# jesselasse/MARL-DMFB

Hardware: AMD Instinct MI355X
Metric: env-steps/sec (whole node), 10x10 DMFB 4-droplet fov9 (higher is better)
Workload: dtype int8 env state/obs + f64 rewards; fp32 Q-net; 1 GPU; DMFB 10x10, drop_num=4, fov=9, 4096 parallel envs per GPU (BASELINE configs[1]); parallelism=dp1: chips sharded per rank, one flat RCCL all-reduce per learn

## Files before the change

### marl_dmfb_amd/csrc/crnn_mfma.h

```cpp
#pragma once
#include <hip/hip_runtime.h>

#include <cstdint>

namespace crnn_mfma {

typedef float f32x4 __attribute__((ext_vector_type(4)));

constexpr int kBlockM = 512;

#ifdef CRNN_PROBE_TS
__device__ unsigned long long *g_crnn_ts;
#define CRNN_TS(k) do { if (lane == 0 && ts_it == 1 && g_crnn_ts) g_crnn_ts[((size_t)blockIdx.x * 8 + wave) * 16 + (k)] = __builtin_readcyclecounter(); } while (0)
#else
#define CRNN_TS(k) do { } while (0)
#endif

template <int OD, int RBV = 0, int NW = 8> struct GeoM {
    static constexpr int RB = RBV ? RBV : (OD <= 24 ? 16 : 12);
    static constexpr int CS = 53;
#ifdef CRNN_NO_ROWLANE
    static constexpr bool ROWLANE = false;
#else
    static constexpr bool ROWLANE = RB == 16;
#endif
    static constexpr int ROW_A1 = ROWLANE ? (OD * CS + 31) / 32 * 32 + 2 : OD * CS;
    static constexpr int IN_STRIDE = ROWLANE ? 258 : 244;
    static constexpr int PAD_COLS = (OD * 25 + 10 + 63) / 64 * 64;
    static constexpr int OUT_STRIDE = PAD_COLS + 4;
    static constexpr int KQ = OD / 4;
    static constexpr int NSTEP2 = KQ * 9;
    static constexpr int M1 = RB * 49, M2 = RB * 25;
    static constexpr int T2 = (M2 + 15) / 16;
    static constexpr int NSUB = NW / 2;
    static constexpr int BLOCK = 64 * NW;
    static_assert(NW == 8 || NW == 4, "wave roles");
    static_assert(RB % NSUB == 0 && RB <= 16, "conv1 tiling: rows split over NSUB waves per half, one position-48 tile");
    static constexpr int VEC = 18;
    static constexpr int MLP = 10 * VEC + 10;
    static constexpr size_t LDS_FLOATS = (size_t)RB * IN_STRIDE + (size_t)RB * ROW_A1 + (size_t)RB * OUT_STRIDE + (size_t)RB * VEC + MLP;
};

template <int OD, int RBV, int NT>
__device__ __forceinline__ void conv2_tiles(const float *s_a1, float *s_out, const float (&bw2)[GeoM<OD, RBV>::NSTEP2], float bias2,
                                            int t0, int t1, int j, int kq, int ch, bool chv) {
    using G = GeoM<OD, RBV>;
    const float *ap[NT];
    f32x4 acc[NT];
#pragma unroll
    for (int n = 0; n < NT; ++n) {
        int r, p;
        if constexpr (G::ROWLANE) {
            r = j;
            p = n == 0 ? t0 : t1;
        } else {
            int m = (n == 0 ? t0 : t1) * 16 + j;
            m = m < G::M2 ? m : G::M2 - 1;
            r = m / 25;
            p = m - r * 25;
        }
        ap[n] = s_a1 + r * G::ROW_A1 + (p / 5) * 7 + p % 5 + kq * G::CS;
        acc[n] = f32x4{bias2, bias2, bias2, bias2};
    }
    float v[2][NT][9];
#pragma unroll
    for (int tap = 0; tap < 9; ++tap)
#pragma unroll
        for (int n = 0; n < NT; ++n) v[0][n][tap] = ap[n][(tap / 3) * 7 + tap % 3];
#ifdef CRNN_PROBE_NO_GATHER
#define CRNN_GATHER(x) (bias2)
#else
#define CRNN_GATHER(x) (x)
#endif
#pragma unroll
    for (int cq = 0; cq < G::KQ; ++cq) {
        if (cq + 1 < G::KQ) {
#pragma unroll
            for (int tap = 0; tap < 9; ++tap)
#pragma unroll
                for (int n = 0; n < NT; ++n)
                    v[(cq + 1) & 1][n][tap] = CRNN_GATHER(ap[n][(cq + 1) * 4 * G::CS + (tap / 3) * 7 + tap % 3]);
        }
        __builtin_amdgcn_sched_barrier(0);
#pragma unroll
        for (int tap = 0; tap < 9; ++tap)
#pragma unroll
            for (int n = 0; n < NT; ++n)
                acc[n] = __builtin_amdgcn_mfma_f32_16x16x4f32(v[cq & 1][n][tap], bw2[cq * 9 + tap], acc[n], 0, 0, 0);
        __builtin_amdgcn_sched_barrier(0);
    }
#ifdef CRNN_PROBE_NO_EPI
    if (chv && acc[0][0] == 12345.678f) {
#else
    if (chv) {
#endif
#pragma unroll
        for (int n = 0; n < NT; ++n)
#pragma unroll
            for (int q = 0; q < 4; ++q) {
                if constexpr (G::ROWLANE) {
                    s_out[(kq * 4 + q) * G::OUT_STRIDE + ch * 25 + (n == 0 ? t0 : t1)] = fmaxf(acc[n][q], 0.0f);
                } else {
                    const int mm = (n == 0 ? t0 : t1) * 16 + kq * 4 + q;
                    if (mm < G::M2) { const int rr = mm / 25, pp = mm - rr * 25; s_out[rr * G::OUT_STRIDE + ch * 25 + pp] = fmaxf(acc[n][q], 0.0f); }
                }
            }
    }
}

template <int OD, int RBV = 0, int NW = 8>
__global__ __launch_bounds__(64 * NW) void k_conv9_mfma(const int8_t *__restrict__ obs, long obs_stride, long rows,
                                                        const float *__restrict__ w1, const float *__restrict__ b1,
                                                        const float *__restrict__ w2, const float *__restrict__ b2,
                                                        float *__restrict__ out, long out_stride, int out_cols,
                                                        const int8_t *__restrict__ onehot, int n_actions,
                                                        const float *__restrict__ mlp_w, const float *__restrict__ mlp_b,
                                                        const int32_t *__restrict__ live_chips, const int32_t *__restrict__ n_live,
                                                        int rows_per_chip) {
    using G = GeoM<OD, RBV, NW>;
    constexpr int kBlockM = G::BLOCK;
    extern __shared__ __attribute__((aligned(16))) float lds[];
    float *s_in = lds;
    float *s_a1 = s_in + G::RB * G::IN_STRIDE;
    float *s_out = s_a1 + G::RB * G::ROW_A1;
    float *s_vec = s_out + G::RB * G::OUT_STRIDE;
    float *s_mlp = s_vec + G::RB * G::VEC;
    const int tid = threadIdx.x, lane = tid & 63, wave = tid >> 6;
    const int nh = (wave >> 1) & 1, sub = (wave & 1) + 2 * (wave >> 2);
    const int j = lane & 15, kq = lane >> 4;
    const int ch = nh * 16 + j;
    const bool chv = ch < OD;

    if (live_chips) rows = min(rows, (long)n_live[0] * rows_per_chip);
    const long n_blocks = (rows + G::RB - 1) / G::RB;
    const int nin = 2 + n_actions;
    if (mlp_w) {
        for (int i = tid; i < 10 * nin; i += kBlockM) s_mlp[i] = mlp_w[i];
        if (tid < 10) s_mlp[10 * G::VEC + tid] = mlp_b[tid];
    }
    const uint32_t rpc = (uint32_t)(rows_per_chip > 0 ? rows_per_chip : 1);
    const uint32_t rpc_magic = rpc > 1 ? (uint32_t)(0x100000000ull / rpc) + 1u : 0u;
    auto src_row = [&](long cr) -> long {
        if (!live_chips) return cr;
        const uint32_t k = rpc > 1 ? __umulhi((uint32_t)cr, rpc_magic) : (uint32_t)cr;
        return (long)((uint32_t)live_chips[k] * rpc + ((uint32_t)cr - k * rpc));
    };
    constexpr int RPW = (G::RB + NW - 1) / NW, ROWB = 245;
    const int wave_u = __builtin_amdgcn_readfirstlane(wave);
    int pf[RPW][4], pfo[RPW];
    int pf_rv = 0;
#pragma unroll
    for (int h = 0; h < RPW; ++h) {
        pfo[h] = 0;
#pragma unroll
        for (int v = 0; v < 4; ++v) pf[h][v] = 0;
    }
    const int p3 = min(lane + 192, mlp_w ? ROWB - 1 : 242);
    auto fetch = [&](long b) {
        const long r0 = b * G::RB;
        pf_rv = b < n_blocks ? (int)min((long)G::RB, rows - r0) : 0;
#pragma unroll
        for (int h = 0; h < RPW; ++h) {
            const int rr = wave_u + NW * h;
            if (rr < pf_rv) {
                const long sr = src_row(r0 + rr);
                const int8_t *row = obs + sr * obs_stride;
                pf[h][0] = row[lane];
                pf[h][1] = row[lane + 64];
                pf[h][2] = row[lane + 128];
                pf[h][3] = row[p3];
                if (mlp_w && onehot && n_actions > 0) pfo[h] = onehot[sr * n_actions + min(lane, n_actions - 1)];
            }
        }
    };
    auto park = [&]() {
#pragma unroll
        for (int h = 0; h < RPW; ++h) {
            const int rr = wave_u + NW * h;
            if (rr < G::RB) {
                const bool on = rr < pf_rv;
                float *dst = s_in + rr * G::IN_STRIDE;
#pragma unroll
                for (int v = 0; v < 3; ++v) dst[lane + 64 * v] = on ? (float)pf[h][v] : 0.0f;
                const float last = on ? (float)pf[h][3] : 0.0f;
                if (lane + 192 < 243) dst[lane + 192] = last;
                else if (lane + 192 < ROWB) s_vec[rr * G::VEC + lane + 192 - 243] = last;
                if (lane < 16) s_vec[rr * G::VEC + 2 + lane] = (on && onehot && lane < n_actions) ? (float)pfo[h] : 0.0f;
            }
        }
    };
    fetch(blockIdx.x);

    for (int i = tid; i < OD * OD * 9; i += kBlockM) s_a1[i] = w2[i];
    for (int i = tid; i < OD * 27; i += kBlockM) s_in[i] = w1[i];
    __syncthreads();
    float bw1[7];
    int off1[7];
#pragma unroll
    for (int s = 0; s < 7; ++s) {
        const int k = 4 * s + kq;
        const bool kv = k < 27;
        bw1[s] = (chv && kv) ? s_in[ch * 27 + k] : 0.0f;
        const int c0 = k / 9, tap = k - c0 * 9;
        off1[s] = kv ? c0 * 81 + (tap / 3) * 9 + tap % 3 : (G::ROWLANE ? 1 : 0);
    }
    int goff[3];
#pragma unroll
    for (int qt = 0; qt < 3; ++qt) { const int p = qt * 16 + j; goff[qt] = (p / 7) * 9 + p % 7; }
    float bw2[G::NSTEP2];
#pragma unroll
    for (int cq = 0; cq < G::KQ; ++cq)
#pragma unroll
        for (int tap = 0; tap < 9; ++tap) bw2[cq * 9 + tap] = chv ? s_a1[(ch * OD + 4 * cq + kq) * 9 + tap] : 0.0f;
    __syncthreads();
    const float bias1 = chv ? b1[ch] : 0.0f, bias2 = chv ? b2[ch] : 0.0f;
    const int n_feat = OD * 25 + (mlp_w ? 10 : 0);
    const int n_out = out_cols > n_feat ? out_cols : n_feat;
    const bool wide_out = (out_stride % 2 == 0) && (((size_t)out) % 8 == 0) && (n_out % 2 == 0);
    const bool quad_out = (out_stride % 4 == 0) && (((size_t)out) % 16 == 0) && (n_out % 4 == 0) && (G::OUT_STRIDE % 4 == 0);
    for (int i = tid; i < G::RB * (G::OUT_STRIDE - n_feat); i += kBlockM) {
        const int rr = i / (G::OUT_STRIDE - n_feat), k = i - rr * (G::OUT_STRIDE - n_feat);
        s_out[rr * G::OUT_STRIDE + n_feat + k] = 0.0f;
    }

    park();
    __syncthreads();
#ifdef CRNN_PROBE_TS
    int ts_it = 0;
#endif
    for (long blk = blockIdx.x; blk < n_blocks; blk += gridDim.x) {
        CRNN_TS(0);
        const long row0 = blk * G::RB;
        const int rv = (int)min((long)G::RB, rows - row0);
        float mv = 0.0f;
        const int mr = tid / 10, mc = tid - mr * 10;
        if (mlp_w && tid < G::RB * 10) {
            mv = s_mlp[10 * G::VEC + mc];
            for (int k = 0; k < nin; ++k) mv = fmaf(s_vec[mr * G::VEC + k], s_mlp[mc * nin + k], mv);
        }
        fetch(blk + gridDim.x);
        CRNN_TS(1);
#ifndef CRNN_PROBE_SKIP_CONV1
        if constexpr (G::ROWLANE) {
            constexpr int NT1 = 49, NIT = (NT1 / G::NSUB) / 3;
            static_assert(G::NSUB == 4 && NIT * 3 * G::NSUB == NT1 - 1, "conv1 row-lane tiling");
            const int sub_u = __builtin_amdgcn_readfirstlane(sub);
            int jb = j * G::IN_STRIDE;
            asm volatile("" : "+v"(jb));
            int lb[7];
#pragma unroll
            for (int s = 0; s < 7; ++s) lb[s] = jb + off1[s];
            auto spos = [&](int m) {
                const int p = sub_u + G::NSUB * m;
                return (p / 7) * 9 + p % 7;
            };
            float cv[2][3][7];
#pragma unroll
            for (int c = 0; c < 3; ++c) {
                const int sp = spos(c);
#pragma unroll
                for (int s = 0; s < 7; ++s) cv[0][c][s] = s_in[lb[s] + sp];
            }
#pragma unroll
            for (int it = 0; it < NIT; ++it) {
                if (it + 1 < NIT) {
#pragma unroll
                    for (int c = 0; c < 3; ++c) {
                        const int sp = spos(3 * (it + 1) + c);
#pragma unroll
                        for (int s = 0; s < 7; ++s) cv[(it + 1) & 1][c][s] = s_in[lb[s] + sp];
                    }
                } else if (sub_u == 0) {
#pragma unroll
                    for (int s = 0; s < 7; ++s) cv[(it + 1) & 1][0][s] = s_in[lb[s] + 60];
                }
                __builtin_amdgcn_sched_barrier(0);
                f32x4 acc[3];
#pragma unroll
                for (int c = 0; c < 3; ++c) acc[c] = f32x4{bias1, bias1, bias1, bias1};
#pragma unroll
                for (int s = 0; s < 7; ++s)
#pragma unroll
                    for (int c = 0; c < 3; ++c) acc[c] = __builtin_amdgcn_mfma_f32_16x16x4f32(cv[it & 1][c][s], bw1[s], acc[c], 0, 0, 0);
                __builtin_amdgcn_sched_barrier(0);
                if (chv) {
#pragma unroll
                    for (int c = 0; c < 3; ++c) {
                        float *dst = s_a1 + kq * 4 * G::ROW_A1 + ch * G::CS + sub_u + G::NSUB * (3 * it + c);
#pragma unroll
                        for (int q = 0; q < 4; ++q) dst[q * G::ROW_A1] = fmaxf(acc[c][q], 0.0f);
                    }
                }
            }
            if (sub_u == 0) {
                f32x4 acc = {bias1, bias1, bias1, bias1};
#pragma unroll
                for (int s = 0; s < 7; ++s) acc = __builtin_amdgcn_mfma_f32_16x16x4f32(cv[NIT & 1][0][s], bw1[s], acc, 0, 0, 0);
                if (chv) {
                    float *dst = s_a1 + kq * 4 * G::ROW_A1 + ch * G::CS + 48;
#pragma unroll
                    for (int q = 0; q < 4; ++q) dst[q * G::ROW_A1] = fmaxf(acc[q], 0.0f);
                }
            }
        } else {
            int gq[3];
#pragma unroll
            for (int qt = 0; qt < 3; ++qt) { gq[qt] = goff[qt] + sub * G::IN_STRIDE; asm volatile("" : "+v"(gq[qt])); }
            float cv[2][3][7];
#pragma unroll
            for (int qt = 0; qt < 3; ++qt)
#pragma unroll
                for (int s = 0; s < 7; ++s) cv[0][qt][s] = s_in[gq[qt] + off1[s]];
#pragma unroll
            for (int i = 0; i < G::RB / G::NSUB; ++i) {
                if (i + 1 < G::RB / G::NSUB) {
#pragma unroll
                    for (int qt = 0; qt < 3; ++qt)
#pragma unroll
                        for (int s = 0; s < 7; ++s)
                            cv[(i + 1) & 1][qt][s] = s_in[G::NSUB * (i + 1) * G::IN_STRIDE + gq[qt] + off1[s]];
                }
                __builtin_amdgcn_sched_barrier(0);
                f32x4 acc[3];
#pragma unroll
                for (int qt = 0; qt < 3; ++qt) acc[qt] = f32x4{bias1, bias1, bias1, bias1};
#pragma unroll
                for (int s = 0; s < 7; ++s)
#pragma unroll
                    for (int qt = 0; qt < 3; ++qt) acc[qt] = __builtin_amdgcn_mfma_f32_16x16x4f32(cv[i & 1][qt][s], bw1[s], acc[qt], 0, 0, 0);
                __builtin_amdgcn_sched_barrier(0);
                if (chv) {
                    float *dst = s_a1 + (sub + G::NSUB * i) * G::ROW_A1 + ch * G::CS + kq * 4;
#pragma unroll
                    for (int qt = 0; qt < 3; ++qt)
#pragma unroll
                        for (int q = 0; q < 4; ++q) dst[qt * 16 + q] = fmaxf(acc[qt][q], 0.0f);
                }
            }
            if (sub == 0) {
                const int rr = j < G::RB ? j : G::RB - 1;
                f32x4 acc = {bias1, bias1, bias1, bias1};
#pragma unroll
                for (int s = 0; s < 7; ++s) acc = __builtin_amdgcn_mfma_f32_16x16x4f32(s_in[rr * G::IN_STRIDE + 60 + off1[s]], bw1[s], acc, 0, 0, 0);
                if (chv) {
#pragma unroll
                    for (int q = 0; q < 4; ++q)
                        if (kq * 4 + q < G::RB) s_a1[(kq * 4 + q) * G::ROW_A1 + ch * G::CS + 48] = fmaxf(acc[q], 0.0f);
                }
            }
        }
#endif
        CRNN_TS(2);
        __syncthreads();
        CRNN_TS(3);
        park();
        CRNN_TS(4);
#ifndef CRNN_PROBE_SKIP_CONV2
        {
            int t = sub;
#ifdef CRNN_PROBE_TS
            int ts_k = 8;
#endif
#pragma unroll 1
            for (; t + G::NSUB < G::T2; t += 2 * G::NSUB) {
                conv2_tiles<OD, RBV, 2>(s_a1, s_out, bw2, bias2, t, t + G::NSUB, j, kq, ch, chv);
#ifdef CRNN_PROBE_TS
                CRNN_TS(ts_k); ++ts_k;
#endif
            }
            if (t < G::T2) conv2_tiles<OD, RBV, 1>(s_a1, s_out, bw2, bias2, t, t, j, kq, ch, chv);
        }
#endif
        if (mlp_w && tid < G::RB * 10) s_out[mr * G::OUT_STRIDE + OD * 25 + mc] = fmaxf(mv, 0.0f);
        CRNN_TS(5);
        __syncthreads();
        CRNN_TS(6);
#ifndef CRNN_PROBE_SKIP_OUT
        if (quad_out) {
            for (int rr = wave; rr < rv; rr += kBlockM / 64) {
                float4 *dst = (float4 *)(out + (row0 + rr) * out_stride);
                const float4 *src = (const float4 *)(s_out + rr * G::OUT_STRIDE);
                for (int k = lane; k < n_out / 4; k += 64) dst[k] = src[k];
            }
        } else if (wide_out) {
            for (int rr = wave; rr < rv; rr += kBlockM / 64) {
                float2 *dst = (float2 *)(out + (row0 + rr) * out_stride);
                const float2 *src = (const float2 *)(s_out + rr * G::OUT_STRIDE);
                for (int k = lane; k < n_out / 2; k += 64) dst[k] = src[k];
            }
        } else {
            for (int rr = wave; rr < rv; rr += kBlockM / 64) {
                float *dst = out + (row0 + rr) * out_stride;
                const float *src = s_out + rr * G::OUT_STRIDE;
                for (int k = lane; k < n_out; k += 64) dst[k] = src[k];
            }
        }
#endif
        CRNN_TS(7);
#ifdef CRNN_PROBE_TS
        ++ts_it;
#endif
    }
}


}
```

Measured before the change: 7.548 million env-steps/s.

## Retile conv2 MFMA work with paired-position tiles for OD=24 rowlane layout

For the OD=24, 8-wave, rowlane geometry, conv2 work is split across waves by kind. Four waves handle channels 0-15 with ordinary 9-tap tiles. The other four pack channels 16-23 into two output positions per lane group, using shifted 12-tap weight windows (horizontal 3x4 or vertical 4x3 patterns). The aim is to fill the 16-wide MFMA columns that were previously half idle for 24 channels. It also adds double-buffered LDS gathers inside the new tile routine, at the cost of more weight registers (KQ*12 per lane) and uneven per-wave workloads.

```diff
diff --git a/marl_dmfb_amd/csrc/crnn_mfma.h b/marl_dmfb_amd/csrc/crnn_mfma.h
--- a/marl_dmfb_amd/csrc/crnn_mfma.h
+++ b/marl_dmfb_amd/csrc/crnn_mfma.h
@@ -24,12 +24,18 @@
 #else
     static constexpr bool ROWLANE = RB == 16;
 #endif
+#ifdef CRNN_NO_PAIRTILE
+    static constexpr bool PAIR = false;
+#else
+    static constexpr bool PAIR = ROWLANE && OD == 24 && NW == 8;
+#endif
     static constexpr int ROW_A1 = ROWLANE ? (OD * CS + 31) / 32 * 32 + 2 : OD * CS;
     static constexpr int IN_STRIDE = ROWLANE ? 258 : 244;
     static constexpr int PAD_COLS = (OD * 25 + 10 + 63) / 64 * 64;
     static constexpr int OUT_STRIDE = PAD_COLS + 4;
     static constexpr int KQ = OD / 4;
     static constexpr int NSTEP2 = KQ * 9;
+    static constexpr int NSTEPX = KQ * 12;
     static constexpr int M1 = RB * 49, M2 = RB * 25;
     static constexpr int T2 = (M2 + 15) / 16;
     static constexpr int NSUB = NW / 2;
@@ -105,6 +111,62 @@
                     if (mm < G::M2) { const int rr = mm / 25, pp = mm - rr * 25; s_out[rr * G::OUT_STRIDE + ch * 25 + pp] = fmaxf(acc[n][q], 0.0f); }
                 }
             }
+    }
+}
+
+template <int OD, int NT, int KIND>
+__device__ __forceinline__ void conv2_rl_tiles(const float *s_a1, float *s_out, const float (&bw)[GeoM<OD>::NSTEPX], float bias, int p0, int p1,
+                                               int col, bool ok, int j, int kq) {
+    using G = GeoM<OD>;
+    static_assert(G::PAIR && (NT == 1 || NT == 2), "pair geometry");
+    constexpr int NTAP = KIND == 0 ? 9 : 12, TW = KIND == 1 ? 4 : 3;
+    const float *ap[NT];
+    f32x4 acc[NT];
+#ifdef CRNN_PROBE_NO_GATHER
+    const float bias2 = bias;
+#endif
+#pragma unroll
+    for (int n = 0; n < NT; ++n) {
+        const int p = n == 0 ? p0 : p1;
+        ap[n] = s_a1 + j * G::ROW_A1 + (p / 5) * 7 + p % 5 + kq * G::CS;
+        acc[n] = f32x4{bias, bias, bias, bias};
+    }
+    constexpr int GS = KIND == 0 ? 9 : 6, GPQ = NTAP / GS, NG = G::KQ * GPQ;
+    auto aoff = [](int g, int i) { const int tap = (g % GPQ) * GS + i; return (g / GPQ) * 4 * G::CS + (tap / TW) * 7 + tap % TW; };
+    float v[2][NT][GS];
+#pragma unroll
+    for (int i = 0; i < GS; ++i)
+#pragma unroll
+        for (int n = 0; n < NT; ++n) v[0][n][i] = ap[n][aoff(0, i)];
+#pragma unroll
+    for (int g = 0; g < NG; ++g) {
+        if (g + 1 < NG) {
+#pragma unroll
+            for (int i = 0; i < GS; ++i)
+#pragma unroll
+                for (int n = 0; n < NT; ++n) v[(g + 1) & 1][n][i] = CRNN_GATHER(ap[n][aoff(g + 1, i)]);
+        }
+        __builtin_amdgcn_sched_barrier(0);
+#pragma unroll
+        for (int i = 0; i < GS; ++i)
+#pragma unroll
+            for (int n = 0; n < NT; ++n) {
+                const int k = (g % GPQ) * GS + i;
+                acc[n] = __builtin_amdgcn_mfma_f32_16x16x4f32(v[g & 1][n][i], bw[(g / GPQ) * 12 + k], acc[n], 0, 0, 0);
+            }
+        __builtin_amdgcn_sched_barrier(0);
+    }
+#ifdef CRNN_PROBE_NO_EPI
+    if (ok && acc[0][0] == 12345.678f) {
+#else
+    if (ok) {
+#endif
+#pragma unroll
+        for (int n = 0; n < NT; ++n) {
+            float *dst = s_out + kq * 4 * G::OUT_STRIDE + col + (n == 0 ? p0 : p1);
+#pragma unroll
+            for (int q = 0; q < 4; ++q) dst[q * G::OUT_STRIDE] = fmaxf(acc[n][q], 0.0f);
+        }
     }
 }
 
@@ -207,13 +269,28 @@
     int goff[3];
 #pragma unroll
     for (int qt = 0; qt < 3; ++qt) { const int p = qt * 16 + j; goff[qt] = (p / 7) * 9 + p % 7; }
-    float bw2[G::NSTEP2];
-#pragma unroll
-    for (int cq = 0; cq < G::KQ; ++cq)
-#pragma unroll
-        for (int tap = 0; tap < 9; ++tap) bw2[cq * 9 + tap] = chv ? s_a1[(ch * OD + 4 * cq + kq) * 9 + tap] : 0.0f;
+    const int wave_r = __builtin_amdgcn_readfirstlane(wave);
+    const int bkind = !G::PAIR || wave_r < 4 ? 0 : wave_r == 5 ? 2 : 1;
+    const int xe = j >> 3, bch = G::PAIR ? (bkind == 0 ? j : 16 + (j & 7)) : ch;
+    float bw2[G::PAIR ? G::NSTEPX : G::NSTEP2];
+    if constexpr (G::PAIR) {
+#pragma unroll
+        for (int cq = 0; cq < G::KQ; ++cq)
+#pragma unroll
+            for (int u = 0; u < 12; ++u) {
+                const int ty = bkind == 1 ? u / 4 : bkind == 2 ? u / 3 - xe : u / 3;
+                const int tx = bkind == 1 ? u % 4 - xe : u % 3;
+                const bool ok = ty >= 0 && ty < 3 && tx >= 0 && tx < 3;
+                bw2[cq * 12 + u] = ok ? s_a1[(bch * OD + 4 * cq + kq) * 9 + ty * 3 + tx] : 0.0f;
+            }
+    } else {
+#pragma unroll
+        for (int cq = 0; cq < G::KQ; ++cq)
+#pragma unroll
+            for (int tap = 0; tap < 9; ++tap) bw2[cq * 9 + tap] = chv ? s_a1[(ch * OD + 4 * cq + kq) * 9 + tap] : 0.0f;
+    }
     __syncthreads();
-    const float bias1 = chv ? b1[ch] : 0.0f, bias2 = chv ? b2[ch] : 0.0f;
+    const float bias1 = chv ? b1[ch] : 0.0f, bias2 = G::PAIR ? b2[bch] : chv ? b2[ch] : 0.0f;
     const int n_feat = OD * 25 + (mlp_w ? 10 : 0);
     const int n_out = out_cols > n_feat ? out_cols : n_feat;
     const bool wide_out = (out_stride % 2 == 0) && (((size_t)out) % 8 == 0) && (n_out % 2 == 0);
@@ -356,7 +433,26 @@
         park();
         CRNN_TS(4);
 #ifndef CRNN_PROBE_SKIP_CONV2
-        {
+        if constexpr (G::PAIR) {
+            const int col = bch * 25 + (bkind == 1 ? xe : bkind == 2 ? 5 * xe : 0);
+            constexpr int T9 = 0, PH = 1, PV = 2;
+            if (wave_r < 4) {
+                const int pa = wave_r < 2 ? 7 * wave_r : wave_r == 2 ? 14 : 20;
+                conv2_rl_tiles<OD, 2, T9>(s_a1, s_out, bw2, bias2, pa, pa + 1, col, true, j, kq);
+                conv2_rl_tiles<OD, 2, T9>(s_a1, s_out, bw2, bias2, pa + 2, pa + 3, col, true, j, kq);
+                if (wave_r < 3) conv2_rl_tiles<OD, 2, T9>(s_a1, s_out, bw2, bias2, pa + 4, pa + 5, col, true, j, kq);
+                if (wave_r != 2) { const int pl = wave_r == 3 ? 24 : pa + 6; conv2_rl_tiles<OD, 1, T9>(s_a1, s_out, bw2, bias2, pl, pl, col, true, j, kq); }
+            } else if (wave_r == 5) {
+                conv2_rl_tiles<OD, 2, PV>(s_a1, s_out, bw2, bias2, 4, 14, col, true, j, kq);
+                conv2_rl_tiles<OD, 1, PV>(s_a1, s_out, bw2, bias2, 19, 19, col, xe == 1, j, kq);
+            } else {
+                const int q0 = wave_r == 4 ? 0 : wave_r == 6 ? 3 : 6;
+                auto pos = [](int q) { return (q >> 1) * 5 + (q & 1) * 2; };
+                conv2_rl_tiles<OD, 2, PH>(s_a1, s_out, bw2, bias2, pos(q0), pos(q0 + 1), col, true, j, kq);
+                if (wave_r == 7) conv2_rl_tiles<OD, 2, PH>(s_a1, s_out, bw2, bias2, pos(q0 + 2), pos(q0 + 3), col, true, j, kq);
+                else conv2_rl_tiles<OD, 1, PH>(s_a1, s_out, bw2, bias2, pos(q0 + 2), pos(q0 + 2), col, true, j, kq);
+            }
+        } else {
             int t = sub;
 #ifdef CRNN_PROBE_TS
             int ts_k = 8;
```

Result: faster. 7.736 million env-steps/s, median of 6 (+2.5%).
